# lambdaloop/ucoslam-cv3

Hardware: AMD Instinct MI355X
Metric: tracking frames/sec (ORB extract + match + local BA), 1241x376 mono (higher is better)
Workload: dtype u8 (ORB, Hamming) + f64 (BA); 1 GPU; orb1241x376_2000f_8lv + hamming_knn_2000x10000_nn10 + local_ba_10kf_3000pt; frames_per_keyframe=4

## Files before the change

### ucoslam-cv3_amd/csrc/ba.hip

```cpp
#include <cfloat>
#include <climits>
#include <limits>
#include <cstdio>
#include <emmintrin.h>
#include <immintrin.h>
#include <condition_variable>
#include <mutex>
#include <string>
#include <thread>
#include <type_traits>
#include <cmath>
#include <cstdlib>
#include <chrono>
#include <atomic>

#include "common.hpp"
#include "reduce.hpp"

namespace {

constexpr int kMaxFree = 64;
constexpr int kThreads = 256;
constexpr int kSolveThreads = 256;
constexpr int kHbmThreads = 512;
// ... 2048 lines not shown
        const int code = mk.slot_edge[i];
        v += mk.blk[cur][(size_t)kMkBlock * (code >> 1) + ((code & 1) ? 42 : 0) + q];
    }
    return v;
}

__global__ __launch_bounds__(64) void ba_mk_assemble_kernel(BAPtrs p, BADims d, BAWide w, BAMarkers mk, int slot) {
    const BAState st = p.st[slot];
    if (st.phase == 2) return;
    const int s = blockIdx.x, q = threadIdx.x;
    const int i0 = mk.slot_ptr[s], i1 = mk.slot_ptr[s + 1];
    if (i0 == i1) return;
    const size_t ld = w.ld;
    if (q < 42) {
        const double v = mk_slot_sum(mk, st.cur, s, q);
        if (q >= 36) { p.bp[6 * s + (q - 36)] += v; w.S[(size_t)d.n * ld + 6 * s + (q - 36)] += v; }
        else { const int a = q / 6, c = q - 6 * a; if (c <= a) w.S[(size_t)(6 * s + a) * ld + 6 * s + c] += v; }
    }
    if (q < 36) {
        const int a = q / 6, c = q - 6 * a;
        for (int i = i0; i < i1; i++) {
            const int code = mk.slot_edge[i];
            if (code & 1) continue;
            const int e = code >> 1, sf = p.slot[mk.e_kf[e]];
            if (sf < 0) continue;
            w.S[(size_t)(6 * s + a) * ld + 6 * sf + c] += mk.blk[st.cur][(size_t)kMkBlock * e + 84 + q];
        }
    }
}

__global__ __launch_bounds__(64) void ba_mk_advance_kernel(BAPtrs p, BADims d, BAMarkers mk, int slot) {
    const int lane = threadIdx.x;
    const BAState st0 = p.st[slot];
    const DecideSums sm = decide_sums(p, mk_decide_dims(d, mk.n_edges), lane, st0.lambda);
    BAState st = (st0.phase != 2 && st0.pending) ? apply_decision(st0, sm, st0.stop_seen != 0) : st0;
    if (st.phase == 2) {
        if (lane == 0) { st.pending = 0; p.st[slot ^ 1] = st; }
        return;
    }
    if (st.iteration == 0 && st.qmax == 0) {
        double m = 0;
        for (int i = lane; i < d.nPointBlocks; i += 64) m = fmax(m, p.part_maxdiag[i]);
        for (int i = lane; i < d.nfree * 6; i += 64) {
            const int s = i / 6, a = i - 6 * s;
            const int q = a * 6 - a * (a - 1) / 2;
            double v = 0;
            for (int c = 0; c < kCamChunks; c++) v += p.HppPart[((size_t)s * kCamChunks + c) * 27 + q];
            v += mk_slot_sum(mk, st.cur, s, 7 * a);
            m = fmax(m, fabs(v));
        }
#pragma unroll
        for (int o = 32; o > 0; o >>= 1) m = fmax(m, __shfl_xor(m, o));
        st.lambda = 1e-5 * m; st.ni = 2;
    }
    if (lane == 0) { BAState pub = st; pub.pending = 1; pub.stop_seen = 0; p.st[slot ^ 1] = pub; }
}

#include "ba_persist.hpp"

}

struct StageLayout {
    size_t pose0, poseR0, intr, slot, free_kf, fix_kf;
    size_t poses_in, fixed, intr_f;
    size_t points, obs;
};
struct ResLayout { size_t poses, state, points, chi2, bad, bytes, bytes_no_chi2; };

constexpr int kKnobUnset = INT_MIN;
struct BAKnobs {
    bool legacy = false;
    bool wide = false;
    int nf = 0;
    int lw = kKnobUnset;
    int nsplit = kKnobUnset;
    bool hbm_solve = false;
    bool prebuilt_off = false;
    bool schur_dense_off = false;
    int dense_g = kKnobUnset;
    bool spec = true;
    bool obs24 = false;
    bool no_avx512 = false;
};
static BAKnobs read_knobs() {
    BAKnobs k;
    const char* e;
    if ((e = getenv("UH_BA_FORM"))) k.legacy = std::string(e) == "legacy";
    if ((e = getenv("UH_BA_WIDE"))) k.wide = atoi(e) != 0;
    if ((e = getenv("UH_BA_NF"))) k.nf = atoi(e);
    if ((e = getenv("UH_BA_LW"))) k.lw = atoi(e);
    if ((e = getenv("UH_BA_NSPLIT"))) k.nsplit = atoi(e);
    if ((e = getenv("UH_BA_SOLVE"))) k.hbm_solve = std::string(e) == "hbm";
    if ((e = getenv("UH_BA_PREBUILT"))) k.prebuilt_off = atoi(e) == 0;
    if ((e = getenv("UH_BA_SCHUR_DENSE"))) k.schur_dense_off = atoi(e) == 0;
    if ((e = getenv("UH_BA_DENSE_G"))) k.dense_g = atoi(e);
    if ((e = getenv("UH_BA_SPEC"))) k.spec = e[0] != '0';
    if ((e = getenv("UH_BA_OBS24"))) k.obs24 = atoi(e) != 0;
    k.no_avx512 = getenv("UH_BA_NO_AVX512") != nullptr;
    return k;
}

struct BALimits { int cus, max_lds; size_t packed_static; };
static void query_limits(const uh_ctx* ctx, BALimits& l) {
    (void)hipSetDevice(ctx->device);
    l.cus = ctx->num_cus > 0 ? ctx->num_cus : 256;
    int v = 0;
    l.max_lds = (hipDeviceGetAttribute(&v, hipDeviceAttributeMaxSharedMemoryPerBlock, ctx->device) == hipSuccess && v > 0) ? v : 64 * 1024;
    hipFuncAttributes fa{};
    l.packed_static = hipFuncGetAttributes(&fa, reinterpret_cast<const void*>(&ba_solve_kernel<false, true>)) == hipSuccess ? fa.sharedSizeBytes : (size_t)1 << 30;
    (void)hipGetLastError();
}

struct PersistPlan { int NF, Lw, G, krows, nelem, SL, max_fix, kfix, lds, nb4, nblk, KS, off_cam; };
enum { kFormChain = 0, kFormPersist = 1, kFormWide = 2 };
enum { kSchurPair, kSchurDense, kSchurDenseWide };
enum { kSolveFused, kSolvePacked, kSolveHbm };
struct BAPlanIn {
    int K, P, E, nfree;
    bool stereo;
    bool persist_ok;
    bool markers;
};
struct BAPlan {
    int form;
    bool persist_candidate;
    PersistPlan ps;
    int nsplit;
    int schur; SchurDense sd; size_t lds_schur;
    int solve; size_t lds_solve;
    int pre_mode;
    bool assemble_pairs;
    int ns_backsub, ns_solve;
};

static bool plan_persist(const BAPlanIn& in, const BAKnobs& kn, const BALimits& lim, PersistPlan& pl) {
    const int nfree = in.nfree, P = in.P;
    const int NF = ((kn.nf == 8 || kn.nf == 16) && nfree <= kn.nf) ? kn.nf : (nfree <= 8 ? 8 : (nfree <= 16 ? 16 : 0));
    if (!NF) return false;
    const int kLwMax = kPThreads / NF;
    int Lw = std::max(std::min(8, kLwMax), std::min(kLwMax, uh_div_up(P, 64)));
    if (kn.lw != kKnobUnset) Lw = std::max(1, std::min(kLwMax, kn.lw));
    const int G = uh_div_up(P, Lw);
    if (G > lim.cus) return false;
    const int kfix = in.K - nfree;
    if (kfix > 255) return false;
    pl.NF = NF; pl.Lw = Lw; pl.G = G; pl.kfix = kfix;
    pl.max_fix = Lw * kfix;
    pl.krows = (3 * Lw + 15) & ~15;
    const int n = 6 * nfree;
    pl.nb4 = (n + 3) / 4; pl.nblk = pl.nb4 * (pl.nb4 + 1) / 2;
    pl.off_cam = pl.nblk * 16;
    pl.nelem = pl.off_cam + NF * 27 + 6 * NF + 4;
    pl.SL = (uh_div_up(pl.nelem, G) + 1) & ~1;
    pl.KS = 1;
    int best = 1 << 30;
    for (int ks = 1; ks <= 6; ks++) {
        if (ks > 1 && ks * pl.off_cam > (n + 1) * (n + 1) + 1452) break;
        const int rounds = uh_div_up(pl.nblk * ks, kPThreads), depth = (uh_div_up(pl.krows, ks) + 3) & ~3;
        if (rounds * depth < best) { best = rounds * depth; pl.KS = ks; }
    }
    pl.lds = NF == 8 ? persist_lds<8>(pl.krows, n, pl.max_fix, pl.kfix, pl.off_cam, pl.KS, pl.SL).total_bytes
                     : persist_lds<16>(pl.krows, n, pl.max_fix, pl.kfix, pl.off_cam, pl.KS, pl.SL).total_bytes;
    return pl.lds <= lim.max_lds;
}

static BAPlan plan_ba(const BAPlanIn& in, const BAKnobs& kn, const BALimits& lim) {
    BAPlan pl{};
    const int nfree = in.nfree, n = 6 * nfree, P = in.P, npairs = nfree * (nfree + 1) / 2;
    pl.persist_candidate = in.persist_ok && !in.stereo && !in.markers && !kn.legacy && !kn.wide && nfree >= 1 && P >= 1 && in.E < (1 << 20) - 1;
    if (pl.persist_candidate && plan_persist(in, kn, lim, pl.ps)) { pl.form = kFormPersist; return pl; }
    pl.form = (nfree > kMaxFree || in.markers || (kn.wide && nfree > 0)) ? kFormWide : kFormChain;
    pl.nsplit = std::max(1, std::min(kMaxSplit, uh_div_up(P, kThreads)));
    if (npairs > 32) pl.nsplit = std::max(1, std::min(pl.nsplit, uh_div_up(300, npairs)));
    if (kn.nsplit != kKnobUnset) pl.nsplit = std::max(1, std::min(kMaxSplit, kn.nsplit));
    if (pl.form == kFormWide) return pl;
    if (nfree >= 17 && !kn.schur_dense_off) {
        SchurDense& sd = pl.sd;
        sd.ntt = uh_div_up(n, 16); sd.T = sd.ntt * (sd.ntt + 1) / 2;
        sd.ys = 16 * sd.ntt + ((sd.ntt & 1) ? 0 : 16);
        const bool widek = nfree > 32;
        const int chunks = std::max(uh_div_up(P, widek ? 8 : 16), 1);
        const int gmax = kn.dense_g != kKnobUnset ? std::max(1, kn.dense_g) : (widek ? 96 : 224);
        sd.cpw = uh_div_up(chunks, gmax); sd.G = uh_div_up(chunks, sd.cpw);
        pl.schur = kSchurDense;
        pl.lds_schur = (size_t)(48 * sd.ys + 48) * sizeof(double);
        if (widek) {
            sd.SP = uh_div_up(sd.T, 80);
            const int need = uh_div_up(uh_div_up(sd.T, sd.SP), 4);
            sd.nown = need <= 12 ? 12 : (need <= 16 ? 16 : 20);
            pl.schur = kSchurDenseWide;
            pl.lds_schur = (size_t)(24 * sd.ys + 24) * sizeof(double);
        }
        pl.nsplit = 1;
    }
    const size_t packed = ((size_t)(n + 1) * (n + 2) / 2 + 2 + kLdltAux) * sizeof(double);
    if (n <= 126 && !kn.hbm_solve) { pl.solve = kSolveFused; pl.lds_solve = (size_t)(n + 1) * (n + 1) * sizeof(double); }
    else if (nfree <= kPackedFree && packed + lim.packed_static <= (size_t)std::max(lim.max_lds, 0) && !kn.hbm_solve) { pl.solve = kSolvePacked; pl.lds_solve = packed; }
    else pl.solve = kSolveHbm;
    if (pl.schur != kSchurPair && !kn.prebuilt_off) pl.pre_mode = pl.solve == kSolvePacked ? 2 : 1;
    pl.assemble_pairs = pl.schur == kSchurPair && pl.solve == kSolveHbm && npairs > 0 && !kn.prebuilt_off;
    pl.ns_backsub = pl.pre_mode ? 0 : pl.nsplit;
    pl.ns_solve = pl.assemble_pairs ? 0 : pl.ns_backsub;
    return pl;
}

struct uh_ba {
    uh_ctx* ctx = nullptr;
    bool have_problem = false;
    BADims dims{};
    BAPtrs ptrs{};
    uh_ba_params params{5, 0.0, 0.0, 1.0f};
    std::vector<float> poses_in;
    std::vector<unsigned char> fixed;
    uh::DevBuf arena;
    uh::DevBuf d_poses_in, d_poses_out, d_points_out, d_bad;
    uh::PinBuf up_pin;
    hipEvent_t ev_up = nullptr; bool up_in_flight = false;
    uh::PinBuf res_pin;
    double* d_pose0 = nullptr; double* d_pts0 = nullptr;
    unsigned char* h_stop = nullptr;
    int iters[2] = {0, 0};
    BAKnobs knobs;
    BALimits lim{};
    BAPlan plan{};
    bool stereo = false; BAStereo sx{};
    std::vector<float> stage_depth, stage_bl;
    int persist_blocked = 0;
    BAPersist pq{};
    uh::DevBuf parena;
    unsigned parena_gen = ~0u;
    unsigned char* h_stage = nullptr;
    size_t h_stage_bytes = 0;
    int cap_K = 0, cap_P = 0, cap_E = 0;
    StageLayout slay{};
    uh::DevBuf dstage;
    hipEvent_t ev_stage = nullptr;
    bool stage_in_flight = false;
    uh::DevBuf dT;
    unsigned stage_gen = 0, problem_stage_gen = 0;
    bool persist_not_resident = false;
    unsigned dT_gen = ~0u, tseq = 0;
    uh::DevBuf dbg_arena;
    uh::DevBuf dscratch;
    unsigned done_base = 0;
    unsigned char* h_res = nullptr;
    size_t h_res_bytes = 0;
    ResLayout rlay{};
    uh::DevBuf d_res;
    bool want_chi2 = true;
    int p_lds_set[2] = {0, 0};
    int job_kind = 0;
    const uh_ba_problem* job_problem = nullptr; uh_ba_problem job_problem_copy{};
    int job_dims[3] = {0, 0, 0};
    uh_ba_params job_params{}; bool job_has_params = false;
    unsigned p_seq = 0;
    BAWide wd{};
    int n_mk = 0;
    BAMarkers mk{};
    int step = 0;
    bool optimized = false;
    std::thread worker;
    std::mutex mu;
    std::condition_variable cv;
    std::atomic<int> job{0};
    int job_rc = 0;
    std::string job_err;
    const volatile uint8_t* job_stop = nullptr;
    ~uh_ba() {
        if (worker.joinable()) {
            { std::lock_guard<std::mutex> lk(mu); job = -1; }
            cv.notify_all();
            worker.join();
        }
        if (h_stop) (void)hipHostFree(h_stop);
        if (h_stage) (void)hipHostFree(h_stage);
        if (h_res) (void)hipHostFree(h_res);
        if (ev_stage) (void)hipEventDestroy(ev_stage);
        if (ev_up) (void)hipEventDestroy(ev_up);
    }
};

namespace {

#define UH_LAUNCH_BA(b, K, grid, block, shmem, ...)                                                            \
    do {                                                                                                       \
        if ((b)->stereo) UH_LAUNCH((b)->ctx, (K<true, BAStereo>), grid, block, shmem, __VA_ARGS__, (b)->sx);   \
        else UH_LAUNCH((b)->ctx, (K<false>), grid, block, shmem, __VA_ARGS__);                                 \
    } while (0)
#define UH_LAUNCH_BA1(b, K, T0, grid, block, shmem, ...)                                                           \
    do {                                                                                                           \
        if ((b)->stereo) UH_LAUNCH((b)->ctx, (K<T0, true, BAStereo>), grid, block, shmem, __VA_ARGS__, (b)->sx);   \
        else UH_LAUNCH((b)->ctx, (K<T0, false>), grid, block, shmem, __VA_ARGS__);                                 \
    } while (0)

void enqueue_wide_ldlt(uh_ctx* ctx, const BAPtrs& p, const BADims& d, const BAWide& W, int run) {
    for (int k0 = 0; k0 < d.n; k0 += kWNB) {
        const int nb = std::min(kWNB, d.n - k0), rows = d.n + 1 - (k0 + nb);
        UH_LAUNCH(ctx, ba_ldlw_diag_kernel, dim3(1), dim3(256), 0, p, W, run, k0, nb);
        UH_LAUNCH(ctx, ba_ldlw_panel_kernel, dim3(uh_div_up(rows, 256)), dim3(256), 0, p, d, W, run, k0, nb);
        const int ntile = uh_div_up(rows, 64);
        if (k0 + nb < d.n) UH_LAUNCH(ctx, ba_ldlw_update_kernel, dim3(ntile * (ntile + 1) / 2), dim3(256), 0, p, d, W, run, k0, nb, ntile);
    }
    for (int k0 = ((d.n - 1) / kWNB) * kWNB; k0 >= 0; k0 -= kWNB) {
        const int nb = std::min(kWNB, d.n - k0);
        UH_LAUNCH(ctx, ba_ldlw_back_kernel, dim3(std::max(uh_div_up(k0, 256), 1)), dim3(256), 0, p, W, run, k0, nb);
    }
}

int enqueue_steps(uh_ba* b, int nsteps, bool pass_start) {
    hipStream_t st = b->ctx->stream;
    const BADims& d = b->dims;
    const BAPlan& pl = b->plan;
    const int npairs = d.nfree * (d.nfree + 1) / 2;
// ... 1284 lines not shown
```

### ucoslam-cv3_amd/csrc/ba_persist.hpp

```cpp
#pragma once

#pragma clang fp contract(fast)

constexpr int kPThreads = 256;
constexpr int kPWaves = kPThreads / 64;
constexpr long long kPTimeoutTicksDefault = 10000000ll;

struct BAPersist {
    int G, Lw, krows, SL, nelem, max_fix, kfix;
    int nb4, nblk, KS;
    int n1, n2, stop_at_begin;
    int speculate;
    unsigned launch_id;
    long long timeout_ticks;
    unsigned tag_base;
    float minChi2;
    const unsigned* T; unsigned tseq;
    const uh_ba_obs* obs;
    int obs16;
    const float* points;
    const float* poses_in;
    const int* fix_kf;
    const double* pose0; const double* poseR0;
    float* r_poses; double* r_state; float* r_points; unsigned char* r_bad; double* r_chi2;
    int want_chi2;
    unsigned long long* r_dev; unsigned long long* r_host; size_t r_words;
    unsigned* done_ctr; unsigned done_base;
    unsigned long long* part;
    unsigned long long* red;
    unsigned long long* partC;
    BAState* host_state;
    unsigned long long* host_done;
    unsigned long long* errw;
};

constexpr int kFxCam = 20;
struct PersistLds {
    int Yt, U, usz, out, wsum, x, bp, bs, bsp, wv, pose, poseR, red, sc, fxchi, fxobs, fxcam, fxact_bytes, fxk_bytes, fxid_bytes, fxptr_bytes, pair_bytes, blk_bytes, flag_bytes, total_bytes;
};
template <int NF>
__host__ __device__ inline PersistLds persist_lds(int krows, int n, int max_fix, int kfix, int off_cam, int KS, int SL) {
    constexpr int NP = 6 * NF, YS = NP + 2;
    PersistLds o;
    int a = 0;
    o.Yt = a; a += krows * YS;
    o.U = a;
    o.usz = (n + 1) * (n + 1) + (n + 1 <= 64 ? 2 * 121 * 6 : 2 * 6 * 128 + 4);
    if (o.usz < KS * off_cam) o.usz = KS * off_cam;
    { const int r = KS * off_cam + (SL > 256 ? SL : 256) + 8; if (o.usz < r) o.usz = r; }
    if (o.usz < kPWaves * NF * 33) o.usz = kPWaves * NF * 33;
    if (o.usz < 2048) o.usz = 2048;
    a += o.usz;
    o.out = a; a += NF * 27 + NP + 4;
    o.wsum = a; a += kPWaves * NF * 33;
    o.x = a; a += NP; o.bp = a; a += NP; o.bs = a; a += NP;
    o.bsp = a; a += kPWaves * NP;
    o.wv = a; a += krows;
    o.pose = a; a += 2 * NF * 7; o.poseR = a; a += 2 * NF * 12;
    o.red = a; a += 16; o.sc = a; a += 8;
    o.fxchi = a; a += max_fix;
    o.fxobs = a; a += 3 * max_fix;
    o.fxcam = a; a += kFxCam * kfix;
    o.fxact_bytes = a * 8;
    int b = o.fxact_bytes + ((max_fix + 15) & ~15);
    o.fxk_bytes = b; b += (max_fix + 15) & ~15;
    o.fxid_bytes = b; b += 4 * ((max_fix + 3) & ~3);
    o.fxptr_bytes = b; b += 4 * (kPThreads / NF + 4);
    o.pair_bytes = b; b += NF * (NF + 1) / 2 * 4;
    b = (b + 15) & ~15;
    o.blk_bytes = b; b += ((NP / 4) * (NP / 4 + 1) / 2 * 2 + 15) & ~15;
    o.flag_bytes = b; b += 16;
    o.total_bytes = b;
    return o;
}

typedef double ba_d2 __attribute__((ext_vector_type(2)));
template <int YS>
__device__ __forceinline__ void schur_item_product(const double* ra, const double* rb, int nrows, double (&acc4)[16]) {
    constexpr int RB = YS * 8;
    static_assert(RB % 16 == 0 && 3 * RB + 16 < 65536, "panel row stride");
    typedef __attribute__((address_space(3))) const double* lds_cptr;
    unsigned pa = (unsigned)(size_t)(lds_cptr)ra, pb = (unsigned)(size_t)(lds_cptr)rb;
    const int ng = nrows >> 2;
    ba_d2 a01[4], a23[4], b01[4], b23[4];
#define UH_SP_READ(u)                                                                                                   \
    asm volatile("ds_read_b128 %0, %4 offset:%6\n\tds_read_b128 %1, %4 offset:%7\n\t"                                  \
                 "ds_read_b128 %2, %5 offset:%6\n\tds_read_b128 %3, %5 offset:%7"                                      \
                 : "=&v"(a01[u]), "=&v"(a23[u]), "=&v"(b01[u]), "=&v"(b23[u])                                          \
                 : "v"(pa), "v"(pb), "n"((u) * RB), "n"((u) * RB + 16))
#define UH_SP_WAIT(cnt, u)                                                                                              \
    do {                                                                                                                \
        asm volatile("s_waitcnt lgkmcnt(" #cnt ")" : "+v"(a01[u]), "+v"(a23[u]), "+v"(b01[u]), "+v"(b23[u]));          \
        __builtin_amdgcn_sched_barrier(0);                                                                              \
    } while (0)
#define UH_SP_FMA(A01, A23, B01, B23)                                                                                   \
    do {                                                                                                                \
        const double av[4] = {(A01).x, (A01).y, (A23).x, (A23).y}, bv[4] = {(B01).x, (B01).y, (B23).x, (B23).y};       \
        _Pragma("unroll") for (int r = 0; r < 4; r++)                                                                   \
            _Pragma("unroll") for (int c = 0; c < 4; c++) acc4[r * 4 + c] = fma(av[r], bv[c], acc4[r * 4 + c]);        \
    } while (0)
#define UH_SP_ROW(cnt, u, refill)                                                                                       \
    do {                                                                                                                \
        UH_SP_WAIT(cnt, u);                                                                                             \
        UH_SP_FMA(a01[u], a23[u], b01[u], b23[u]);                                                                      \
        __builtin_amdgcn_sched_barrier(0);                                                                              \
        if (refill) UH_SP_READ(u);                                                                                      \
    } while (0)
    if (ng > 0) {
        UH_SP_READ(0); UH_SP_READ(1); UH_SP_READ(2); UH_SP_READ(3);
        for (int g = 1; g < ng; g++) {
            pa += 4 * RB; pb += 4 * RB;
            UH_SP_ROW(12, 0, true); UH_SP_ROW(12, 1, true); UH_SP_ROW(12, 2, true); UH_SP_ROW(12, 3, true);
        }
        UH_SP_ROW(12, 0, false); UH_SP_ROW(8, 1, false); UH_SP_ROW(4, 2, false); UH_SP_ROW(0, 3, false);
    }
    for (int k = 4 * ng; k < nrows; k++) {
        const ba_d2 ta01 = *reinterpret_cast<const ba_d2*>(ra + k * YS), ta23 = *reinterpret_cast<const ba_d2*>(ra + k * YS + 2);
        const ba_d2 tb01 = *reinterpret_cast<const ba_d2*>(rb + k * YS), tb23 = *reinterpret_cast<const ba_d2*>(rb + k * YS + 2);
        UH_SP_FMA(ta01, ta23, tb01, tb23);
    }
#undef UH_SP_ROW
#undef UH_SP_FMA
#undef UH_SP_WAIT
#undef UH_SP_READ
}

typedef unsigned long long pword;
struct TWord { pword lo, hi; };
__device__ __forceinline__ void tst(pword* base, size_t i, double v, unsigned tag) {
    const pword b = (pword)__double_as_longlong(v);
    typedef unsigned int u32x4 __attribute__((ext_vector_type(4)));
    const u32x4 w = {(unsigned)b, tag, (unsigned)(b >> 32), tag};
    const __amdgpu_buffer_rsrc_t rs = __builtin_amdgcn_make_buffer_rsrc(base, 0, 0x7FFFFFFF, 0x00020000);
    __builtin_amdgcn_raw_buffer_store_b128(w, rs, (int)(i * 16), 0, 16);
}
typedef __amdgpu_buffer_rsrc_t trsrc_t;
__device__ __forceinline__ trsrc_t trsrc(const pword* base) { return __builtin_amdgcn_make_buffer_rsrc(const_cast<pword*>(base), 0, 0x7FFFFFFF, 0x00020000); }
__device__ __forceinline__ void tpoll_begin() { asm volatile("" ::: "memory"); }
__device__ __forceinline__ TWord tld_raw(trsrc_t rs, size_t i) {
    typedef unsigned int u32x4 __attribute__((ext_vector_type(4)));
    const u32x4 r = __builtin_amdgcn_raw_buffer_load_b128(rs, (int)(i * 16), 0, 16);
    TWord w;
    w.lo = (pword)r.x | ((pword)r.y << 32);
    w.hi = (pword)r.z | ((pword)r.w << 32);
    return w;
}
__device__ __forceinline__ bool tok(const TWord& w, unsigned tag) { return (unsigned)(w.lo >> 32) == tag && (unsigned)(w.hi >> 32) == tag; }
__device__ __forceinline__ double tval(const TWord& w) { return __longlong_as_double((long long)((w.hi << 32) | (w.lo & 0xffffffffull))); }

__device__ __forceinline__ double rsqrt_nr(double x) {
    double r = __builtin_amdgcn_rsq(x);
    r = r * fma(-0.5 * x, r * r, 1.5);
    r = r * fma(-0.5 * x, r * r, 1.5);
    return r;
}

template <int JAC>
__device__ __forceinline__ void edge_eval_p(double u, double v, double w, double fx, double fy, double cx, double cy, double delta, double dsqr,
                                            const double* Rt, const double* X, bool robust, EdgeLin& o) {
    const double x = Rt[0] * X[0] + Rt[1] * X[1] + Rt[2] * X[2] + Rt[9];
    const double y = Rt[3] * X[0] + Rt[4] * X[1] + Rt[5] * X[2] + Rt[10];
    const double z = Rt[6] * X[0] + Rt[7] * X[1] + Rt[8] * X[2] + Rt[11];
    const double iz = fast_rcp(z);
    const double xz = x * iz, yz = y * iz;
    o.ex = u - (xz * fx + cx);
    o.ey = v - (yz * fy + cy);
    o.chi2 = w * (o.ex * o.ex + o.ey * o.ey);
    o.rho1 = 1.0;
    o.robchi = o.chi2;
    if (robust && o.chi2 > dsqr) {
        const double rs = rsqrt_nr(o.chi2);
        o.rho1 = delta * rs;
        o.robchi = 2 * (o.chi2 * rs) * delta - dsqr;
    }
    if (JAC >= 1) {
        o.ww = o.rho1 * w;
        o.r0 = -w * o.ex * o.rho1;
        o.r1 = -w * o.ey * o.rho1;
        const double fxz = fx * iz, fyz = fy * iz;
#pragma unroll
        for (int c = 0; c < 3; c++) {
            o.A[c] = -fxz * (Rt[c] - xz * Rt[6 + c]);
            o.A[3 + c] = -fyz * (Rt[3 + c] - yz * Rt[6 + c]);
        }
        if (JAC >= 2) {
            o.B[0] = xz * yz * fx; o.B[1] = -(1 + xz * xz) * fx; o.B[2] = yz * fx; o.B[3] = -fxz; o.B[4] = 0; o.B[5] = xz * fxz;
            o.B[6] = (1 + yz * yz) * fy; o.B[7] = -xz * yz * fy; o.B[8] = -xz * fy; o.B[9] = 0; o.B[10] = -fyz; o.B[11] = yz * fyz;
        }
    }
}

__device__ __forceinline__ void quat_norm_pos_p(double (&q)[4]) {
    if (q[3] < 0) { q[0] = -q[0]; q[1] = -q[1]; q[2] = -q[2]; q[3] = -q[3]; }
    const double rn = rsqrt_nr(q[0] * q[0] + q[1] * q[1] + q[2] * q[2] + q[3] * q[3]);
    q[0] *= rn; q[1] *= rn; q[2] *= rn; q[3] *= rn;
}
__device__ __forceinline__ void quat_from_R_p(const double (&R)[9], double (&q)[4]) {
    const double tr = R[0] + R[4] + R[8];
    if (tr > 0) {
        const double x = tr + 1.0, r = rsqrt_nr(x), h = 0.5 * r;
        q[3] = 0.5 * (x * r);
        q[0] = (R[7] - R[5]) * h; q[1] = (R[2] - R[6]) * h; q[2] = (R[3] - R[1]) * h;
    } else if (!(R[4] > R[0]) && !(R[8] > R[0])) {
        const double x = R[0] - R[4] - R[8] + 1.0, r = rsqrt_nr(x), h = 0.5 * r;
        q[0] = 0.5 * (x * r);
        q[3] = (R[7] - R[5]) * h; q[1] = (R[3] + R[1]) * h; q[2] = (R[6] + R[2]) * h;
    } else if (R[4] > R[0] && !(R[8] > R[4])) {
        const double x = R[4] - R[8] - R[0] + 1.0, r = rsqrt_nr(x), h = 0.5 * r;
        q[1] = 0.5 * (x * r);
        q[3] = (R[2] - R[6]) * h; q[2] = (R[7] + R[5]) * h; q[0] = (R[1] + R[3]) * h;
    } else {
        const double x = R[8] - R[0] - R[4] + 1.0, r = rsqrt_nr(x), h = 0.5 * r;
        q[2] = 0.5 * (x * r);
        q[3] = (R[3] - R[1]) * h; q[0] = (R[2] + R[6]) * h; q[1] = (R[5] + R[7]) * h;
    }
}
__device__ __forceinline__ void se3_left_update_p(double (&q)[4], double (&t)[3], const double* dx) {
    const double w0 = dx[0], w1 = dx[1], w2 = dx[2];
    const double th2 = w0 * w0 + w1 * w1 + w2 * w2;
    const double O[9] = {0, -w2, w1, w2, 0, -w0, -w1, w0, 0};
    double O2[9];
#pragma unroll
    for (int r = 0; r < 3; r++)
#pragma unroll
        for (int c = 0; c < 3; c++) O2[r * 3 + c] = O[r * 3] * O[c] + O[r * 3 + 1] * O[3 + c] + O[r * 3 + 2] * O[6 + c];
    double a, b, c2;
    if (!(th2 >= 1e-10)) { a = 1; b = 0.5; c2 = 1.0 / 6.0; }
    else {
        const double rth = rsqrt_nr(th2), theta = th2 * rth, rth2 = rth * rth;
        double sn, cs;
        sincos(theta, &sn, &cs);
        a = sn * rth; b = (1 - cs) * rth2; c2 = (theta - sn) * (rth2 * rth);
    }
    double Rm[9], V[9];
#pragma unroll
    for (int i = 0; i < 9; i++) { const double I = (i % 4 == 0) ? 1.0 : 0.0; Rm[i] = I + a * O[i] + b * O2[i]; V[i] = I + b * O[i] + c2 * O2[i]; }
    double qe[4];
    quat_from_R_p(Rm, qe);
    quat_norm_pos_p(qe);
    double te[3];
#pragma unroll
    for (int r = 0; r < 3; r++) te[r] = V[r * 3] * dx[3] + V[r * 3 + 1] * dx[4] + V[r * 3 + 2] * dx[5];
    double RE[9];
    quat_to_R(qe, RE);
    double qn[4];
    qn[3] = qe[3] * q[3] - qe[0] * q[0] - qe[1] * q[1] - qe[2] * q[2];
    qn[0] = qe[3] * q[0] + qe[0] * q[3] + qe[1] * q[2] - qe[2] * q[1];
    qn[1] = qe[3] * q[1] + qe[1] * q[3] + qe[2] * q[0] - qe[0] * q[2];
    qn[2] = qe[3] * q[2] + qe[2] * q[3] + qe[0] * q[1] - qe[1] * q[0];
    double tn[3];
#pragma unroll
    for (int r = 0; r < 3; r++) tn[r] = RE[r * 3] * t[0] + RE[r * 3 + 1] * t[1] + RE[r * 3 + 2] * t[2] + te[r];
    quat_norm_pos_p(qn);
#pragma unroll
    for (int i = 0; i < 4; i++) q[i] = qn[i];
#pragma unroll
    for (int i = 0; i < 3; i++) t[i] = tn[i];
}


template <int W>
__device__ __forceinline__ double group_sum(double v) {
    v += dpp_f64<kDppXor1>(v);
    v += dpp_f64<kDppXor2>(v);
    v += dpp_f64<kDppHalfMirror>(v);
    if (W >= 16) v += dpp_f64<kDppMirror>(v);
    if (W >= 32) { double a = v, b = v; swap_rows<16>(a, b); v = a + b; }
    if (W >= 64) { double a = v, b = v; swap_rows<32>(a, b); v = a + b; }
    return v;
}
template <int W>
__device__ __forceinline__ double group_max(double v) {
    v = fmax(v, dpp_f64<kDppXor1>(v));
    v = fmax(v, dpp_f64<kDppXor2>(v));
    v = fmax(v, dpp_f64<kDppHalfMirror>(v));
    if (W >= 16) v = fmax(v, dpp_f64<kDppMirror>(v));
    if (W >= 32) { double a = v, b = v; swap_rows<16>(a, b); v = fmax(a, b); }
// ... 223 lines not shown
            tpoll_begin();
            TWord w[8];
#pragma unroll
            for (int u = 0; u < 8; u++) if ((todo >> u) & 1u) w[u] = tld_raw(rs, first + u * stride);
#pragma unroll
            for (int u = 0; u < 8; u++) if (((todo >> u) & 1u) && tok(w[u], tag)) { v[u] = tval(w[u]); todo &= ~(1u << u); }
            if (!todo || give_up(t0)) return;
        }
    };
    const unsigned sl_inv = (unsigned)(0x100000000ull / (unsigned)SL) + 1u;
    auto div_sl = [&](int i) -> int { return (int)__umulhi((unsigned)i, sl_inv); };
    auto part_at = [&](int i) -> size_t { const int sl = div_sl(i); return ((size_t)sl * G + g) * SL + (i - sl * SL); };

    auto prod_index = [&](int row, int col) -> int {
        const int bi = row >> 2, bj = col >> 2;
        return (bi * q.nb4 - bi * (bi - 1) / 2 + (bj - bi)) * 16 + (row & 3) * 4 + (col & 3);
    };
    auto is_diag_elem = [&](int idx) -> bool {
        if (idx >= OFF_CAM) return false;
        int row, col;
        const int bq = idx >> 4;
        row = 4 * s_blk[bq][0] + ((idx >> 2) & 3); col = 4 * s_blk[bq][1] + (idx & 3);
        return row == col && col < n;
    };
    int fold_i[2], fold_s[2];
#pragma unroll
    for (int u = 0; u < 2; u++) {
        const int t = tid + u * kPThreads;
        fold_i[u] = -1; fold_s[u] = 0;
        if (t < nfree * 21) {
            const int sc = t / 21, qq = t - 21 * sc;
            int a = 0, rem = qq;
            while (rem >= 6 - a) { rem -= 6 - a; ++a; }
            fold_i[u] = prod_index(6 * sc + a, 6 * sc + a + rem);
            fold_s[u] = sc * 27 + qq;
        }
    }
    const bool red_diag0 = tid < SL && is_diag_elem(g * SL + tid);
    const int open_beg = div_sl(OFF_CAM) * SL;
    const int red_HG = max(1, min(G, kPThreads / SL));
    const unsigned hg_inv = (unsigned)(0x100000000ull / (unsigned)red_HG) + 1u;
    bool clk_on = false;
    int n_kept = 0, n_dropped = 0;
#define UH_BA_CLKT(i) do { if (clk_on) UH_BA_CLK(i); } while (0)
    BAState st;
    memset(&st, 0, sizeof(st));
    st.phase = 2; st.lambda = -1; st.ni = 2;
    bool robust = true;
    double chi_lin_pass = 0;

    double acc[10];
    double hp[33];
    double H[18];
    bool any = false;
    auto lin_eval = [&](int buf, const double (&Xp)[3], bool first) {
#pragma unroll
        for (int i = 0; i < 10; i++) acc[i] = 0;
#pragma unroll
        for (int i = 0; i < 33; i++) hp[i] = 0;
#pragma unroll
        for (int i = 0; i < 18; i++) H[i] = 0;
        any = false;
        const bool on = has && act;
        if (on) {
            EdgeLin L;
            edge_eval_p<2>(ou, ov, ow, fxk, fyk, cxk, cyk, d.delta, d.dsqr, s_poseR + (buf * NF + s) * 12, Xp, robust, L);
            any = true;
            if (first) chi_e = L.chi2;
            acc[9] = L.robchi;
            acc[0] = L.ww * (L.A[0] * L.A[0] + L.A[3] * L.A[3]); acc[1] = L.ww * (L.A[0] * L.A[1] + L.A[3] * L.A[4]);
            acc[2] = L.ww * (L.A[0] * L.A[2] + L.A[3] * L.A[5]); acc[3] = L.ww * (L.A[1] * L.A[1] + L.A[4] * L.A[4]);
            acc[4] = L.ww * (L.A[1] * L.A[2] + L.A[4] * L.A[5]); acc[5] = L.ww * (L.A[2] * L.A[2] + L.A[5] * L.A[5]);
            acc[6] = L.A[0] * L.r0 + L.A[3] * L.r1; acc[7] = L.A[1] * L.r0 + L.A[4] * L.r1; acc[8] = L.A[2] * L.r0 + L.A[5] * L.r1;
#pragma unroll
            for (int a = 0; a < 6; a++)
#pragma unroll
                for (int c = 0; c < 3; c++) H[a * 3 + c] = L.ww * (L.B[a] * L.A[c] + L.B[6 + a] * L.A[3 + c]);
            int qq = 0;
#pragma unroll
            for (int a = 0; a < 6; a++)
#pragma unroll
                for (int c = a; c < 6; c++) hp[qq++] = L.ww * (L.B[a] * L.B[c] + L.B[6 + a] * L.B[6 + c]);
#pragma unroll
            for (int a = 0; a < 6; a++) hp[21 + a] = L.B[a] * L.r0 + L.B[6 + a] * L.r1;
        }
        {
            for (int i = fxb + s; i < fxe; i += NF) {
                if (!s_fxact[i]) continue;
                any = true;
                const double* C = s_fxcam + kFxCam * s_fxk[i];
                EdgeLin L;
                edge_eval_p<1>(s_fxobs[3 * i], s_fxobs[3 * i + 1], s_fxobs[3 * i + 2], C[12], C[13], C[14], C[15], d.delta, d.dsqr, C, Xp, robust, L);
                if (first) s_fxchi[i] = L.chi2;
                acc[9] += L.robchi;
                acc[0] += L.ww * (L.A[0] * L.A[0] + L.A[3] * L.A[3]); acc[1] += L.ww * (L.A[0] * L.A[1] + L.A[3] * L.A[4]);
                acc[2] += L.ww * (L.A[0] * L.A[2] + L.A[3] * L.A[5]); acc[3] += L.ww * (L.A[1] * L.A[1] + L.A[4] * L.A[4]);
                acc[4] += L.ww * (L.A[1] * L.A[2] + L.A[4] * L.A[5]); acc[5] += L.ww * (L.A[2] * L.A[2] + L.A[5] * L.A[5]);
                acc[6] += L.A[0] * L.r0 + L.A[3] * L.r1; acc[7] += L.A[1] * L.r0 + L.A[4] * L.r1; acc[8] += L.A[2] * L.r0 + L.A[5] * L.r1;
            }
        }
    };
    auto phase1 = [&](double lambda, bool first, double scale_lane, double stop_val) {
        tagA = next_tag();
        if (!first) UH_BA_CLKT(52);
#pragma unroll
        for (int i = 0; i < 10; i++) acc[i] = group_sum<NF>(acc[i]);
        const unsigned long long anym = __ballot(any);
        any_pt = ((anym >> (lane & ~(NF - 1))) & ((1ull << NF) - 1)) != 0;
        bl0 = acc[6]; bl1 = acc[7]; bl2 = acc[8];
        if (first) {
        } else if (any_pt) {
            const double d00 = acc[0] + lambda, d11 = acc[3] + lambda, d22 = acc[5] + lambda;
            ci00 = rsqrt_nr(d00);
            cl10 = acc[1] * ci00; cl20 = acc[2] * ci00;
            ci11 = rsqrt_nr(d11 - cl10 * cl10);
            cl21 = (acc[4] - cl20 * cl10) * ci11;
            ci22 = rsqrt_nr(d22 - cl20 * cl20 - cl21 * cl21);
            wl0 = bl0 * ci00;
            wl1 = (bl1 - cl10 * wl0) * ci11;
            wl2 = (bl2 - cl20 * wl0 - cl21 * wl1) * ci22;
        } else {
            ci00 = ci11 = ci22 = cl10 = cl20 = cl21 = wl0 = wl1 = wl2 = 0;
        }
        if (!first && 3 * ll + 2 < q.krows) {
#pragma unroll
            for (int a = 0; a < 6; a++) {
                const double y0 = H[a * 3] * ci00;
                const double y1 = (H[a * 3 + 1] - cl10 * y0) * ci11;
                const double y2 = (H[a * 3 + 2] - cl20 * y0 - cl21 * y1) * ci22;
                Yt[(3 * ll) * YS + 6 * s + a] = y0; Yt[(3 * ll + 1) * YS + 6 * s + a] = y1; Yt[(3 * ll + 2) * YS + 6 * s + a] = y2;
                hp[27 + a] = y0 * wl0 + y1 * wl1 + y2 * wl2;
            }
        }
        {
            int off = 0, real = 33;
            PartTranspose<33, 32, NF>::run(hp, lane, off, real);
#pragma unroll
            for (int i = 0; i < NHP; i++) if (i < real) s_wsum[(wv * NF + s) * 33 + off + i] = hp[i];
        }
        if (!first) UH_BA_CLKT(53);
        const double chi_part = (live && s == 0) ? acc[9] : 0.0;
        const double maxd = (live && s == 0 && any_pt) ? fmax(fabs(acc[0]), fmax(fabs(acc[3]), fabs(acc[5]))) : 0.0;
        double cs = chi_part, mx = maxd, ss = scale_lane;
        block_reduce3<kPWaves>(cs, mx, ss, s_red);
        for (int t = tid; t < NF * 33; t += kPThreads) {
            double r = s_wsum[t];
#pragma unroll
            for (int w = 1; w < kPWaves; w++) r += s_wsum[w * NF * 33 + t];
            const int sc = t / 33, i = t - 33 * sc;
            s_out[i < 27 ? sc * 27 + i : NF * 27 + 6 * sc + (i - 27)] = r;
        }
        if (tid == 0) { s_out[NF * 27 + NP] = cs; s_out[NF * 27 + NP + 1] = ss; s_out[NF * 27 + NP + 2] = mx; s_out[NF * 27 + NP + 3] = g == 0 ? stop_val : 0.0; }
        if (!first) UH_BA_CLKT(54);
        if (!first) {
            const int nitems = q.nblk * q.KS;
            const int kc = (q.krows + q.KS - 1) / q.KS;
            for (int item = tid; item < nitems; item += kPThreads) {
                const int kt = item / q.nblk, bq = item - kt * q.nblk;
                const int bi = s_blk[bq][0], bj = s_blk[bq][1];
                const int kbeg = kt * kc, kend = min(q.krows, kbeg + kc);
                double acc4[16];
#pragma unroll
                for (int i = 0; i < 16; i++) acc4[i] = 0;
                schur_item_product<YS>(Yt + kbeg * YS + 4 * bi, Yt + kbeg * YS + 4 * bj, kend - kbeg, acc4);
#pragma unroll
                for (int i = 0; i < 16; i++) U[kt * OFF_CAM + bq * 16 + i] = acc4[i];
            }
        }
        if (!first) UH_BA_CLKT(55);
        __syncthreads();
        if (!first) UH_BA_CLKT(56);
        if (!first) {
#pragma unroll
            for (int u = 0; u < 2; u++) if (fold_i[u] >= 0) U[fold_i[u]] -= s_out[fold_s[u]];
            for (int j = tid; j < n; j += kPThreads) { const int sc = j / 6; s_out[NF * 27 + j] -= s_out[sc * 27 + 21 + (j - 6 * sc)]; }
        }
        __syncthreads();
        if (!first) UH_BA_CLKT(60);
        for (int i = tid; i < NF * 27 + NP + 4; i += kPThreads) {
            if (!first && i < NF * 27 && i - 27 * (i / 27) < 21) continue;
            tst(q.part, part_at(OFF_CAM + i), s_out[i], tagA);
        }
        if (!first) UH_BA_CLKT(61);
        const int KSs = q.KS;
        for (int i = (first ? open_beg : 0) + tid; i < OFF_CAM; i += kPThreads) {
            double r = 0.0;
            if (!first) { r = U[i]; for (int kt = 1; kt < KSs; kt++) r += U[kt * OFF_CAM + i]; }
            tst(q.part, part_at(i), r, tagA);
        }
    };

    unsigned tagB = 0;
    auto reduce_slices = [&](double lam, bool first) -> bool {
        tagB = next_tag();
        const int HG = red_HG;
        double* const R = U + q.KS * OFF_CAM;
        const size_t src = (size_t)g * G * SL;
        for (int idx = tid; idx < SL * HG; idx += kPThreads) {
            const int hg = div_sl(idx), e = idx - hg * SL;
            const bool is_max = g * SL + e == OFF_SC + 2;
            const int ge = g * SL + e;
            const bool hpp = ge >= OFF_CAM && ge < OFF_BS && (ge - OFF_CAM) - 27 * ((ge - OFF_CAM) / 27) < 21;
            const bool used = ge < q.nelem && !(first && (g + 1) * SL <= OFF_CAM) && !(hpp && !first);
            double r = 0.0;
            bool have = false;
            for (int h = hg; used && h < G; h += 8 * HG) {
                double v[8];
                const int cnt = min(8, HG == 1 ? G - h : (int)__umulhi((unsigned)(G - h + HG - 1), hg_inv));
                tload8(rs_part, src + (size_t)h * SL + e, (size_t)HG * SL, cnt, tagA, v);
#pragma unroll
                for (int u = 0; u < 8; u++) {
                    if (u >= cnt) continue;
                    r = !have ? v[u] : (is_max ? fmax(r, v[u]) : r + v[u]);
                    have = true;
                }
            }
            R[idx] = r;
        }
        UH_BA_CLKT(50);
        __syncthreads();
        if (s_flag[1]) return false;
        for (int e = tid; e < SL; e += kPThreads) {
            const bool is_max = g * SL + e == OFF_SC + 2;
            double r = R[e];
            for (int hg = 1; hg < HG; hg++) { const double v = R[hg * SL + e]; r = is_max ? fmax(r, v) : r + v; }
            if (e == tid ? red_diag0 : is_diag_elem(g * SL + e)) r -= lam;
            {
                const int ge = g * SL + e;
                if (!first && ge >= OFF_CAM && ge < OFF_BS && (ge - OFF_CAM) - 27 * ((ge - OFF_CAM) / 27) < 21) continue;
            }
            tst(q.red, (size_t)g * SL + e, r, tagB);
        }
        UH_BA_CLKT(51);
        __syncthreads();
        return true;
    };

    auto dst_of = [&](int idx) -> int {
        int t = -1;
        if (idx < q.nelem) {
            if (idx < OFF_CAM) {
                int row, col;
                const int bq = idx >> 4, rr = (idx >> 2) & 3, cq = idx & 3;
                row = 4 * s_blk[bq][0] + rr; col = 4 * s_blk[bq][1] + cq;
                if (row <= col && col < n) t = o.U + col * ld + row;
            } else if (idx < OFF_BS) {
                const int i = idx - OFF_CAM, sc = i / 27, k = i - 27 * sc;
                if (k >= 21) t = (o.bp + 6 * sc + (k - 21)) | (1 << 24);
            } else if (idx < OFF_SC) t = o.U + n * ld + (idx - OFF_BS);
            else t = (o.sc + 4 + (idx - OFF_SC)) | (1 << 24);
        }
        return t;
    };
    int asm_dst[8];
#pragma unroll
    for (int u = 0; u < 8; u++) asm_dst[u] = dst_of(tid + u * kPThreads);
    UH_BA_CLK(1);
    for (int pass = 0; pass < 2; pass++) {
        UH_BA_CLK(2 + 3 * pass);
        if (pass == 1) {
            if (st.stopped) break;
            st.gate = 1;
            st.iters_pass1 = st.iters_done;
            if (has) {
                const double* Rt = s_poseR + (st.cur * NF + s) * 12;
                const double z = Rt[6] * X[0] + Rt[7] * X[1] + Rt[8] * X[2] + Rt[11];
                if (chi_e > d.chi2_th || !(z > 0.0)) act = false;
            }
            for (int i = fxb + s; i < fxe; i += NF) {
                const double* Rt = s_fxcam + kFxCam * s_fxk[i];
                const double z = Rt[6] * X[0] + Rt[7] * X[1] + Rt[8] * X[2] + Rt[11];
                if (s_fxchi[i] > d.chi2_th || !(z > 0.0)) s_fxact[i] = 0;
            }
            robust = false;
            __syncthreads();
        }
        const int max_iters = pass == 0 ? q.n1 : q.n2;
        st.pending = 0; st.stop_seen = 0;
        st.phase = max_iters > 0 ? 0 : 2;
        st.iteration = 0; st.max_iters = max_iters; st.qmax = 0; st.solve_ok = 1; st.first_trial = 1; st.iters_done = 0;
        st.prevChi2 = FLT_MAX; st.curChi2 = FLT_MAX; st.minChi2 = q.minChi2;
        if (pass == 0 && q.stop_at_begin) { st.phase = 2; st.stopped = 1; }
        if (st.phase == 2) continue;

        bool opening = true;
        bool pend = false;
        double lambda_spec = 0, scale_lane = 0, stop_val = 0;
        int loop_no = 0;
        while (opening || st.phase != 2) {
            ++loop_no;
            clk_on = pass == 1 && loop_no == 4;
            double lambda = pend ? lambda_spec : st.lambda;
            int cur = st.cur, trial = cur ^ 1;
            UH_BA_CLKT(40);
            if (g == 0 && tid == 64 && p.stop)
                __builtin_amdgcn_global_load_lds((__attribute__((address_space(1))) const void*)const_cast<const unsigned char*>(p.stop),
                                                 (__attribute__((address_space(3))) void*)(s_flag + 2), 4, 0, 0);
            {
                const double Xe[3] = {pend ? Xt[0] : X[0], pend ? Xt[1] : X[1], pend ? Xt[2] : X[2]};
                lin_eval(pend ? trial : cur, Xe, opening || pend);
                phase1(opening ? 1.0 : lambda, opening, scale_lane, stop_val);
            }
            UH_BA_CLKT(41);
            if (!reduce_slices(opening ? 0.0 : lambda, opening)) return;
            UH_BA_CLKT(42);
            if (opening) {
                opening = false;
                double m = 0.0;
                {
                    const int d0 = lane, d1 = lane + 64;
                    const int sc0 = d0 / 6, a0 = d0 - 6 * sc0, sc1 = d1 / 6, a1 = d1 - 6 * sc1;
                    const size_t i_d0 = d0 < n ? (size_t)(OFF_CAM + sc0 * 27 + (a0 * 6 - a0 * (a0 - 1) / 2)) : (size_t)OFF_SC;
                    const size_t i_d1 = d1 < n ? (size_t)(OFF_CAM + sc1 * 27 + (a1 * 6 - a1 * (a1 - 1) / 2)) : (size_t)OFF_SC;
                    long long t0 = 0;
                    for (;;) {
                        tpoll_begin();
                        const TWord wm = tld_raw(rs_red, OFF_SC + 2), wd0 = tld_raw(rs_red, i_d0), wd1 = tld_raw(rs_red, i_d1), wc = tld_raw(rs_red, OFF_SC);
                        m = lane == 0 ? tval(wm) : 0.0;
                        if (d0 < n) m = fmax(m, fabs(tval(wd0)));
                        if (d1 < n) m = fmax(m, fabs(tval(wd1)));
                        chi_lin_pass = tval(wc);
// ... 262 lines not shown
```

Before: 9696 frames/s.

## Compute persistent BA Schur product with f64 MFMA tiles instead of scalar FMAs

After: 9904 frames/s, median of 6. +2.2%, better.

```diff
diff --git a/ucoslam-cv3_amd/csrc/ba.hip b/ucoslam-cv3_amd/csrc/ba.hip
--- a/ucoslam-cv3_amd/csrc/ba.hip
+++ b/ucoslam-cv3_amd/csrc/ba.hip
@@ -2224,13 +2224,7 @@
     pl.off_cam = pl.nblk * 16;
     pl.nelem = pl.off_cam + NF * 27 + 6 * NF + 4;
     pl.SL = (uh_div_up(pl.nelem, G) + 1) & ~1;
-    pl.KS = 1;
-    int best = 1 << 30;
-    for (int ks = 1; ks <= 6; ks++) {
-        if (ks > 1 && ks * pl.off_cam > (n + 1) * (n + 1) + 1452) break;
-        const int rounds = uh_div_up(pl.nblk * ks, kPThreads), depth = (uh_div_up(pl.krows, ks) + 3) & ~3;
-        if (rounds * depth < best) { best = rounds * depth; pl.KS = ks; }
-    }
+    pl.KS = schur_mfma_splits(uh_div_up(n, 16));
     pl.lds = NF == 8 ? persist_lds<8>(pl.krows, n, pl.max_fix, pl.kfix, pl.off_cam, pl.KS, pl.SL).total_bytes
                      : persist_lds<16>(pl.krows, n, pl.max_fix, pl.kfix, pl.off_cam, pl.KS, pl.SL).total_bytes;
     return pl.lds <= lim.max_lds;
diff --git a/ucoslam-cv3_amd/csrc/ba_persist.hpp b/ucoslam-cv3_amd/csrc/ba_persist.hpp
--- a/ucoslam-cv3_amd/csrc/ba_persist.hpp
+++ b/ucoslam-cv3_amd/csrc/ba_persist.hpp
@@ -74,55 +74,89 @@
     return o;
 }
 
-typedef double ba_d2 __attribute__((ext_vector_type(2)));
-template <int YS>
-__device__ __forceinline__ void schur_item_product(const double* ra, const double* rb, int nrows, double (&acc4)[16]) {
-    constexpr int RB = YS * 8;
-    static_assert(RB % 16 == 0 && 3 * RB + 16 < 65536, "panel row stride");
+typedef double ba_f64x4 __attribute__((ext_vector_type(4)));
+template <int YS, int NTT, int WV, bool KSPLIT>
+__device__ __forceinline__ void schur_mfma_tiles(const double* Yt, int k4beg, int k4end, double* Uw, int nb4, int lane) {
+    constexpr int TT = NTT * (NTT + 1) / 2, NOWN = KSPLIT ? TT : (TT - WV + 3) / 4, T0 = KSPLIT ? 0 : WV, TS = KSPLIT ? 1 : 4;
+    static_assert(NOWN >= 1 && 16 * NTT <= YS, "tile list / panel row");
+    const int i16 = lane & 15, kq = lane >> 4;
+    ba_f64x4 acc[NOWN];
     typedef __attribute__((address_space(3))) const double* lds_cptr;
-    unsigned pa = (unsigned)(size_t)(lds_cptr)ra, pb = (unsigned)(size_t)(lds_cptr)rb;
-    const int ng = nrows >> 2;
-    ba_d2 a01[4], a23[4], b01[4], b23[4];
-#define UH_SP_READ(u)                                                                                                   \
-    asm volatile("ds_read_b128 %0, %4 offset:%6\n\tds_read_b128 %1, %4 offset:%7\n\t"                                  \
-                 "ds_read_b128 %2, %5 offset:%6\n\tds_read_b128 %3, %5 offset:%7"                                      \
-                 : "=&v"(a01[u]), "=&v"(a23[u]), "=&v"(b01[u]), "=&v"(b23[u])                                          \
-                 : "v"(pa), "v"(pb), "n"((u) * RB), "n"((u) * RB + 16))
-#define UH_SP_WAIT(cnt, u)                                                                                              \
-    do {                                                                                                                \
-        asm volatile("s_waitcnt lgkmcnt(" #cnt ")" : "+v"(a01[u]), "+v"(a23[u]), "+v"(b01[u]), "+v"(b23[u]));          \
-        __builtin_amdgcn_sched_barrier(0);                                                                              \
-    } while (0)
-#define UH_SP_FMA(A01, A23, B01, B23)                                                                                   \
-    do {                                                                                                                \
-        const double av[4] = {(A01).x, (A01).y, (A23).x, (A23).y}, bv[4] = {(B01).x, (B01).y, (B23).x, (B23).y};       \
-        _Pragma("unroll") for (int r = 0; r < 4; r++)                                                                   \
-            _Pragma("unroll") for (int c = 0; c < 4; c++) acc4[r * 4 + c] = fma(av[r], bv[c], acc4[r * 4 + c]);        \
-    } while (0)
-#define UH_SP_ROW(cnt, u, refill)                                                                                       \
-    do {                                                                                                                \
-        UH_SP_WAIT(cnt, u);                                                                                             \
-        UH_SP_FMA(a01[u], a23[u], b01[u], b23[u]);                                                                      \
-        __builtin_amdgcn_sched_barrier(0);                                                                              \
-        if (refill) UH_SP_READ(u);                                                                                      \
-    } while (0)
-    if (ng > 0) {
-        UH_SP_READ(0); UH_SP_READ(1); UH_SP_READ(2); UH_SP_READ(3);
-        for (int g = 1; g < ng; g++) {
-            pa += 4 * RB; pb += 4 * RB;
-            UH_SP_ROW(12, 0, true); UH_SP_ROW(12, 1, true); UH_SP_ROW(12, 2, true); UH_SP_ROW(12, 3, true);
-        }
-        UH_SP_ROW(12, 0, false); UH_SP_ROW(8, 1, false); UH_SP_ROW(4, 2, false); UH_SP_ROW(0, 3, false);
-    }
-    for (int k = 4 * ng; k < nrows; k++) {
-        const ba_d2 ta01 = *reinterpret_cast<const ba_d2*>(ra + k * YS), ta23 = *reinterpret_cast<const ba_d2*>(ra + k * YS + 2);
-        const ba_d2 tb01 = *reinterpret_cast<const ba_d2*>(rb + k * YS), tb23 = *reinterpret_cast<const ba_d2*>(rb + k * YS + 2);
-        UH_SP_FMA(ta01, ta23, tb01, tb23);
-    }
-#undef UH_SP_ROW
-#undef UH_SP_FMA
-#undef UH_SP_WAIT
-#undef UH_SP_READ
+    unsigned pa = (unsigned)(size_t)(lds_cptr)(Yt + (4 * k4beg + kq) * YS + i16);
+    double opA[NTT], opB[NTT];
+    auto rd = [&](double (&x)[NTT]) {
+#pragma unroll
+        for (int cg = 0; cg < NTT; cg++) asm volatile("ds_read_b64 %0, %1 offset:%2" : "=&v"(x[cg]) : "v"(pa), "n"(128 * cg));
+    };
+    auto wait_for = [&](double (&x)[NTT]) {
+#pragma unroll
+        for (int cg = 0; cg < NTT; cg++) asm volatile("s_waitcnt lgkmcnt(0)" : "+v"(x[cg]));
+    };
+    auto step = [&](double (&x)[NTT], double (&y)[NTT], unsigned adv, bool first) {
+        wait_for(x);
+#pragma unroll
+        for (int u = 0; u < NOWN; u++) {
+            const double a = x[schur_tile_col(T0 + TS * u)], b = x[schur_tile_row(T0 + TS * u)];
+            if (first) {
+                if (u == 0) asm volatile("s_nop 1\n\tv_mfma_f64_16x16x4_f64 %0, %1, %2, 0" : "=&v"(acc[u]) : "v"(a), "v"(b));
+                else asm volatile("v_mfma_f64_16x16x4_f64 %0, %1, %2, 0" : "=&v"(acc[u]) : "v"(a), "v"(b));
+            } else {
+                if (u == 0) asm volatile("s_nop 1\n\tv_mfma_f64_16x16x4_f64 %0, %1, %2, %0" : "+v"(acc[u]) : "v"(a), "v"(b));
+                else asm volatile("v_mfma_f64_16x16x4_f64 %0, %1, %2, %0" : "+v"(acc[u]) : "v"(a), "v"(b));
+            }
+            if (u == 0) {
+                pa += adv;
+                rd(y);
+            }
+        }
+    };
+    constexpr unsigned RB4 = 4 * YS * 8;
+    const int ks = k4end - k4beg;
+    rd(opA);
+    step(opA, opB, 1 < ks ? RB4 : 0u, true);
+    int sdone = 1;
+    for (; sdone + 2 <= ks; sdone += 2) {
+        step(opB, opA, RB4, false);
+        step(opA, opB, sdone + 2 < ks ? RB4 : 0u, false);
+    }
+    if (sdone < ks) { step(opB, opA, 0u, false); wait_for(opA); }
+    else wait_for(opB);
+    asm volatile("s_nop 15\n\ts_nop 15" : "+v"(acc[0]));
+#pragma unroll
+    for (int u = 1; u < NOWN; u++) asm volatile("" : "+v"(acc[u]));
+    int lo = lane;
+    asm volatile("" : "+v"(lo));
+    const int bjl = (lo & 15) >> 2;
+    double* const Ul = Uw + (bjl * 16 + (lo >> 4) * 4 + (lo & 3));
+#pragma unroll
+    for (int u = 0; u < NOWN; u++) {
+        const int ti = schur_tile_col(T0 + TS * u), tj = schur_tile_row(T0 + TS * u);
+#pragma unroll
+        for (int reg = 0; reg < 4; reg++) {
+            const int bi = 4 * ti + reg;
+            if ((ti < tj || reg <= bjl) && 4 * tj + bjl < nb4) Ul[(bi * nb4 - bi * (bi - 1) / 2 - bi + 4 * tj) * 16] = acc[u][reg];
+        }
+    }
+}
+__host__ __device__ constexpr int schur_mfma_splits(int ntt) { return ntt <= 3 ? kPWaves : 1; }
+template <int NF>
+__device__ __forceinline__ void schur_product_mfma(const double* Yt, int krows, int ntt, double* U, int off_cam, int nb4, int wv, int lane) {
+    constexpr int YS = 6 * NF + 2;
+    const int k4 = krows >> 2, ks = krows >> 4;
+    switch (ntt) {
+    case 1: schur_mfma_tiles<YS, 1, 0, true>(Yt, wv * ks, wv * ks + ks, U + wv * off_cam, nb4, lane); break;
+    case 2: schur_mfma_tiles<YS, 2, 0, true>(Yt, wv * ks, wv * ks + ks, U + wv * off_cam, nb4, lane); break;
+    case 3: schur_mfma_tiles<YS, 3, 0, true>(Yt, wv * ks, wv * ks + ks, U + wv * off_cam, nb4, lane); break;
+    default:
+        if constexpr (NF == 16) {
+#define UH_SCHUR_MFMA_NTT(N) case N: switch (wv) { \
+            case 0: schur_mfma_tiles<YS, N, 0, false>(Yt, 0, k4, U, nb4, lane); break; case 1: schur_mfma_tiles<YS, N, 1, false>(Yt, 0, k4, U, nb4, lane); break; \
+            case 2: schur_mfma_tiles<YS, N, 2, false>(Yt, 0, k4, U, nb4, lane); break; default: schur_mfma_tiles<YS, N, 3, false>(Yt, 0, k4, U, nb4, lane); break; } break;
+            switch (ntt) { UH_SCHUR_MFMA_NTT(4) UH_SCHUR_MFMA_NTT(5) default: UH_SCHUR_MFMA_NTT(6) }
+#undef UH_SCHUR_MFMA_NTT
+        }
+        break;
+    }
 }
 
 typedef unsigned long long pword;
@@ -652,21 +686,8 @@
         }
         if (tid == 0) { s_out[NF * 27 + NP] = cs; s_out[NF * 27 + NP + 1] = ss; s_out[NF * 27 + NP + 2] = mx; s_out[NF * 27 + NP + 3] = g == 0 ? stop_val : 0.0; }
         if (!first) UH_BA_CLKT(54);
-        if (!first) {
-            const int nitems = q.nblk * q.KS;
-            const int kc = (q.krows + q.KS - 1) / q.KS;
-            for (int item = tid; item < nitems; item += kPThreads) {
-                const int kt = item / q.nblk, bq = item - kt * q.nblk;
-                const int bi = s_blk[bq][0], bj = s_blk[bq][1];
-                const int kbeg = kt * kc, kend = min(q.krows, kbeg + kc);
-                double acc4[16];
-#pragma unroll
-                for (int i = 0; i < 16; i++) acc4[i] = 0;
-                schur_item_product<YS>(Yt + kbeg * YS + 4 * bi, Yt + kbeg * YS + 4 * bj, kend - kbeg, acc4);
-#pragma unroll
-                for (int i = 0; i < 16; i++) U[kt * OFF_CAM + bq * 16 + i] = acc4[i];
-            }
-        }
+        if (!first)
+            schur_product_mfma<NF>(Yt, q.krows, (n + 15) >> 4, U, OFF_CAM, q.nb4, wvu, lane);
         if (!first) UH_BA_CLKT(55);
         __syncthreads();
         if (!first) UH_BA_CLKT(56);
```
